# nikizadehgfdl/ocean_model_grid_generator

Measured on AMD Instinct MI355X. Metric: supergrid cells/sec (coords+metrics), 1/8° tripolar at 1/2/4/8 MI355X, higher is better.
Workload: dtype f64

## Files before the change

### include/ogg_hip.h

```cpp
#ifndef OGG_HIP_H
#define OGG_HIP_H

#ifdef __cplusplus
extern "C" {
#endif

#define OGG_OK 0
#define OGG_EORDER 1
#define OGG_ESHAPE 2
#define OGG_EHIP 3
#define OGG_ENOMEM 4
#define OGG_EARG 5

#define OGG_DP_ARC_LITERAL 0
#define OGG_DP_ARC_CHORD 1

#define OGG_SYM_DEFAULT 0
#define OGG_SYM_MIRROR 1
#define OGG_SYM_NONE 2

const char* ogg_last_error(void);
const char* ogg_version(void);
long ogg_abi_sizeof(int which);
int ogg_device_count(int* count);
int ogg_set_device(int device);
int ogg_device_name(char* buf, int buflen);


int ogg_y_mercator_rounded(long Ni, long n, const double* phi_rad, long long* ystar);
int ogg_y_mercator_rounded_dev(long Ni, long n, const double* phi_rad, long long* ystar, void* stream);

int ogg_y_mercator(long Ni, long n, const double* phi_rad, double* y);
int ogg_y_mercator_dev(long Ni, long n, const double* phi_rad, double* y, void* stream);

int ogg_phi_mercator(long Ni, long n, const double* y, double* phi_deg);
int ogg_phi_mercator_dev(long Ni, long n, const double* y, double* phi_deg, void* stream);
int ogg_mercator_axis_dev(long Ni, long long y0, long n, double* phi_deg, void* stream);

int ogg_linear_axis_dev(long n, double a0, double len, double denom, double* out, void* stream);

int ogg_affine_index(long n, const double* idx, double a0, double len, double denom, double* out);
int ogg_affine_index_dev(long n, const double* idx, double a0, double len, double denom, double* out, void* stream);

int ogg_tile_latlon(long nrows, long ni1, const double* lat1d, const double* lon1d, double* x, double* y);
int ogg_tile_latlon_dev(long nrows, long ni1, const double* lat1d, const double* lon1d, double* x, double* y,
                        void* stream);

int ogg_generate_latlon_grid(long lni, long lnj, double llon0, double llen_lon, double llat0, double llen_lat,
                             int skip_first_row, double* x, double* y);


int ogg_mdist(long n, const double* x1, const double* x2, double* out);
int ogg_mdist_dev(long n, const double* x1, const double* x2, double* out, void* stream);

int ogg_grid_metrics_midas_dev(long nrows_xy, long ni1, const double* x, const double* y, long n_pt_rows,
                               long n_cell_rows, double Re, int latlon_areafix, double* dx, double* dy,
                               double* area, double* angle, void* stream);
int ogg_grid_metrics_midas(long nj1, long ni1, const double* x, const double* y, double Re, int latlon_areafix,
                           double* dx, double* dy, double* area);
int ogg_angle_x(long nj1, long ni1, const double* x, const double* y, double* angle_dx);

typedef struct {
    int axis_kind;
    double a0, len, denom;
    long long y0;
    const double* lat1d;
    long k0;
    long n_pt_rows;
    long n_cell_rows;
    double *x, *y, *dx, *dy, *area, *angle;
} ogg_latlon_band;
int ogg_latlon_supergrid_multi_dev(int n_bands, const ogg_latlon_band* bands, long ni1, double lon0, double lenlon, double Re,
                                   int metrics, void* stream);
long ogg_latlon_rows_workspace_bytes(int n_bands, const ogg_latlon_band* bands, long ni1);
int ogg_latlon_supergrid_rows_ws_dev(int n_bands, const ogg_latlon_band* bands, long ni1, double lon0, double lenlon, double Re,
                                     int metrics, void* workspace, long workspace_bytes, void* stream);
int ogg_latlon_supergrid_dev(long n_pt_rows, long n_cell_rows, long ni1, const double* lat1d, const double* lon1d, double Re,
                             int metrics, double* x, double* y, double* dx, double* dy, double* area, double* angle,
                             void* stream);


int ogg_bipolar_projection(long n, const double* lamg, const double* phig, double lon_bp, double rp,
                           int metrics_only, double* lams, double* phis, double* h_i_inv, double* h_j_inv);
int ogg_bipolar_projection_dev(long n, const double* lamg, const double* phig, double lon_bp, double rp,
                               int metrics_only, double* lams, double* phis, double* h_i_inv, double* h_j_inv,
                               void* stream);

int ogg_bipolar_cap_mesh_dev(long Ni, long Nj, double lat0_bp, double lon_bp, long j0, long nrows, double* lams,
                             double* phis, double* h_i_inv, double* h_j_inv, void* stream);
int ogg_bipolar_cap_mesh_angle_dev(long Ni, long Nj, double lat0_bp, double lon_bp, long j0, long nrows, double* lams,
                                   double* phis, double* h_i_inv, double* h_j_inv, double* angle_dx, void* stream);
int ogg_bipolar_cap_mesh_angle_sym_dev(long Ni, long Nj, double lat0_bp, double lon_bp, long j0, long nrows, int symmetry, double* lams,
                                       double* phis, double* h_i_inv, double* h_j_inv, double* angle_dx, void* stream);
int ogg_bipolar_cap_mesh(long Ni, long Nj, double lat0_bp, double lon_bp, double* lams, double* phis,
                         double* h_i_inv, double* h_j_inv);
int ogg_bipolar_cap_mesh_sym(long Ni, long Nj, double lat0_bp, double lon_bp, int symmetry, double* lams, double* phis,
                             double* h_i_inv, double* h_j_inv);

int ogg_bipolar_cap_ij_array(long n_i, const double* i, long n_j, const double* j, long Ni, long Nj, double lat0_bp,
                             double lon_bp, double rp, double* h_i_inv, double* h_j_inv);
int ogg_bipolar_cap_ij_array_dev(long n_i, const double* i, long n_j, const double* j, long Ni, long Nj, double lat0_bp,
                                 double lon_bp, double rp, double* h_i_inv, double* h_j_inv, void* stream);

int ogg_bipolar_cap_metrics_quad_dev(int order, long nx, long ny, double lat0_bp, double lon_bp, double rp,
                                     double Re, long j0, long n_dx_rows, long n_cell_rows, double* dxq, double* dyq,
                                     double* daq, void* stream);
int ogg_bipolar_cap_metrics_quad(int order, long nx, long ny, double lat0_bp, double lon_bp, double rp, double Re,
                                 double* dxq, double* dyq, double* daq);
int ogg_bipolar_cap_metrics_quad_sym(int order, long nx, long ny, double lat0_bp, double lon_bp, double rp, double Re, int symmetry,
                                     double* dxq, double* dyq, double* daq);
long ogg_bipolar_quad_workspace_bytes(int order, long nx, long ny);
int ogg_bipolar_cap_metrics_quad_ws_dev(int order, long nx, long ny, double lat0_bp, double lon_bp, double rp, double Re,
                                        long j0, long n_dx_rows, long n_cell_rows, double* dxq, double* dyq, double* daq,
                                        void* workspace, long workspace_bytes, void* stream);
int ogg_bipolar_cap_metrics_quad_sym_ws_dev(int order, long nx, long ny, double lat0_bp, double lon_bp, double rp, double Re,
                                            long j0, long n_dx_rows, long n_cell_rows, int symmetry, double* dxq, double* dyq, double* daq,
                                            void* workspace, long workspace_bytes, void* stream);

typedef struct ogg_bipolar_band {
    long Ni, Nj;
    double lat0_bp, lon_bp;
    double rp, Re;
    int order;
    int symmetry;
    long j0;
    long n_pt_rows;
    long n_cell_rows;
    double *x, *y, *angle, *dx, *dy, *area;
    void* workspace;
// ... 474 lines not shown
```

### ocean_model_grid_generator_amd/_lib.py

```python
import ctypes
import os

import numpy as np

_HERE = os.path.dirname(os.path.abspath(__file__))
LIB_PATH = os.environ.get("OGG_LIB_PATH") or os.path.join(_HERE, "csrc", "libogg_hip.so")

OGG_OK, OGG_EORDER, OGG_ESHAPE, OGG_EHIP, OGG_ENOMEM, OGG_EARG = 0, 1, 2, 3, 4, 5
DP_ARC_LITERAL, DP_ARC_CHORD = 0, 1
SYM_DEFAULT, SYM_MIRROR, SYM_NONE = 0, 1, 2

MATH = {"div_pi180": 0, "rcp_c3": 1, "rsqrt_c3": 2, "atan_series14": 3, "atan_series17": 4, "atan_cap": 5, "atan2_angle": 6,
        "wave_prev": 7, "wave_next": 8, "wave_prev_tail": 9, "wave_next_tail": 10, "xcd_contiguous": 11, "lib_atan": 12, "atan_lib": 13, "wave_next_int": 14,
        "sin_tiny": 32, "asin_tiny": 33, "cos_cap": 34, "hom_arc": 35, "hom_tan": 36, "lib_sin": 37, "lib_asin": 38, "lib_cos": 39}

c_long, c_int, c_double, c_void_p, c_longlong = ctypes.c_long, ctypes.c_int, ctypes.c_double, ctypes.c_void_p, ctypes.c_longlong
_dp = ctypes.POINTER(ctypes.c_double)
_llp = ctypes.POINTER(ctypes.c_longlong)

class LatlonBand(ctypes.Structure):
    _fields_ = [("axis_kind", c_int), ("a0", c_double), ("len", c_double), ("denom", c_double), ("y0", c_longlong),
                ("lat1d", c_void_p), ("k0", c_long), ("n_pt_rows", c_long), ("n_cell_rows", c_long), ("x", c_void_p),
                ("y", c_void_p), ("dx", c_void_p), ("dy", c_void_p), ("area", c_void_p), ("angle", c_void_p)]

# ... 227 lines not shown
                                         c_void_p, c_void_p, c_void_p, c_void_p],
    "ogg_bipolar_cap_metrics_quad_ws_dev": [c_int, c_long, c_long, c_double, c_double, c_double, c_double, c_long, c_long, c_long,
                                            c_void_p, c_void_p, c_void_p, c_void_p, c_long, c_void_p],
    "ogg_bipolar_cap_metrics_quad_sym_ws_dev": [c_int, c_long, c_long, c_double, c_double, c_double, c_double, c_long, c_long, c_long, c_int,
                                                c_void_p, c_void_p, c_void_p, c_void_p, c_long, c_void_p],
    "ogg_bipolar_cap_metrics_quad": [c_int, c_long, c_long, c_double, c_double, c_double, c_double, c_void_p, c_void_p,
                                     c_void_p],
    "ogg_displaced_pole_mesh_dev": [c_long, c_void_p, c_long, c_void_p, c_long, c_long, c_double, c_double, c_double,
                                    c_double, c_void_p, c_void_p, c_void_p],
    "ogg_displaced_pole_mesh": [c_long, c_void_p, c_long, c_void_p, c_long, c_long, c_double, c_double, c_double, c_double,
                                c_void_p, c_void_p],
    "ogg_displaced_pole_grid_dev": [c_long, c_long, c_double, c_double, c_double, c_double, c_long, c_long, c_void_p,
                                    c_void_p, c_void_p],
    "ogg_displaced_pole_numerical_h_dev": [c_long, c_void_p, c_long, c_void_p, c_long, c_long, c_double, c_double, c_double,
                                           c_double, c_double, c_int, c_void_p, c_void_p, c_void_p],
    "ogg_displaced_pole_numerical_h": [c_long, c_void_p, c_long, c_void_p, c_long, c_long, c_double, c_double, c_double,
                                       c_double, c_double, c_int, c_void_p, c_void_p],
    "ogg_displaced_pole_metrics_quad_dev": [c_int, c_long, c_long, c_double, c_double, c_double, c_double, c_double, c_long,
                                            c_long, c_long, c_void_p, c_void_p, c_void_p, c_void_p],
    "ogg_displaced_pole_metrics_quad_ws_dev": [c_int, c_long, c_long, c_double, c_double, c_double, c_double, c_double, c_long,
                                               c_long, c_long, c_void_p, c_void_p, c_void_p, c_void_p, c_long, c_void_p],
    "ogg_displaced_pole_metrics_quad": [c_int, c_long, c_long, c_double, c_double, c_double, c_double, c_double, c_void_p,
                                        c_void_p, c_void_p],
    "ogg_displaced_pole_metrics_quad_form": [c_int, c_int, c_long, c_long, c_double, c_double, c_double, c_double, c_double, c_void_p,
                                             c_void_p, c_void_p],
    "ogg_displaced_pole_metrics_quad_form_ws_dev": [c_int, c_int, c_long, c_long, c_double, c_double, c_double, c_double, c_double,
                                                    c_long, c_long, c_long, c_void_p, c_void_p, c_void_p, c_void_p, c_long, c_void_p],
    "ogg_displaced_pole_metrics_quad_form_sym_ws_dev": [c_int, c_int, c_int, c_long, c_long, c_double, c_double, c_double, c_double, c_double,
                                                        c_long, c_long, c_long, c_void_p, c_void_p, c_void_p, c_void_p, c_long, c_void_p],
    "ogg_displaced_pole_grid_angle_ws_dev": [c_long, c_long, c_double, c_double, c_double, c_double, c_long, c_long, c_void_p,
                                             c_void_p, c_void_p, c_void_p, c_long, c_void_p],
    "ogg_workspace_error_flag_dev": [c_void_p, ctypes.POINTER(c_int), c_void_p],
    "ogg_y_mercator": [c_long, c_long, c_void_p, c_void_p],
    "ogg_y_mercator_dev": [c_long, c_long, c_void_p, c_void_p, c_void_p],
    "ogg_affine_index": [c_long, c_void_p, c_double, c_double, c_double, c_void_p],
    "ogg_affine_index_dev": [c_long, c_void_p, c_double, c_double, c_double, c_void_p, c_void_p],
    "ogg_mdist": [c_long, c_void_p, c_void_p, c_void_p],
    "ogg_mdist_dev": [c_long, c_void_p, c_void_p, c_void_p, c_void_p],
    "ogg_haversine": [c_long, c_void_p, c_void_p, c_void_p, c_void_p, c_void_p],
    "ogg_haversine_dev": [c_long, c_void_p, c_void_p, c_void_p, c_void_p, c_void_p, c_void_p],
    "ogg_bipolar_cap_ij_array": [c_long, c_void_p, c_long, c_void_p, c_long, c_long, c_double, c_double, c_double, c_void_p,
                                 c_void_p],
    "ogg_bipolar_cap_ij_array_dev": [c_long, c_void_p, c_long, c_void_p, c_long, c_long, c_double, c_double, c_double,
                                     c_void_p, c_void_p, c_void_p],
    "ogg_displaced_pole_projection": [c_long, c_long, c_void_p, c_void_p, c_double, c_double, c_double, c_double, c_void_p,
                                      c_void_p],
    "ogg_displaced_pole_projection_dev": [c_long, c_long, c_void_p, c_void_p, c_double, c_double, c_double, c_double,
                                          c_void_p, c_void_p, c_void_p],
    "ogg_monotonic_bounding": [c_long, c_long, c_void_p, c_double],
    "ogg_monotonic_bounding_dev": [c_long, c_long, c_void_p, c_double, c_void_p],
    "ogg_latlon_supergrid_multi_dev": [c_int, ctypes.POINTER(LatlonBand), c_long, c_double, c_double, c_double, c_int, c_void_p],
    "ogg_latlon_supergrid_rows_ws_dev": [c_int, ctypes.POINTER(LatlonBand), c_long, c_double, c_double, c_double, c_int, c_void_p, c_long,
                                         c_void_p],
    "ogg_tripolar_pass_dev": [c_int, ctypes.POINTER(LatlonBand), c_long, c_double, c_double, c_double, c_int,
                              ctypes.POINTER(BipolarBand), c_void_p],
    "ogg_tripolar_pass_events_dev": [c_int, ctypes.POINTER(LatlonBand), c_long, c_double, c_double, c_double, c_int,
                                     ctypes.POINTER(BipolarBand), ctypes.POINTER(c_void_p), ctypes.POINTER(c_double), c_void_p],
    "ogg_supergrid_pass_dev": [c_int, ctypes.POINTER(LatlonBand), c_long, c_double, c_double, c_double, c_int,
                               ctypes.POINTER(BipolarBand), ctypes.POINTER(DpoleBand), ctypes.POINTER(c_void_p), ctypes.POINTER(c_double),
                               c_void_p],
    "ogg_supergrid_pass_plan_dev": [c_int, ctypes.POINTER(LatlonBand), c_long, c_double, c_double, c_double, c_int,
                                    ctypes.POINTER(BipolarBand), ctypes.POINTER(DpoleBand), ctypes.POINTER(c_void_p)],
    "ogg_supergrid_pass_run_dev": [c_void_p, ctypes.POINTER(c_void_p), ctypes.POINTER(c_double), c_void_p],
    "ogg_supergrid_pass_plan_destroy": [c_void_p],
    "ogg_supergrid_pass_plan_flags_dev": [c_void_p, ctypes.POINTER(c_int), c_void_p],
    "ogg_latlon_supergrid_dev": [c_long, c_long, c_long, c_void_p, c_void_p, c_double, c_int, c_void_p, c_void_p, c_void_p,
                                 c_void_p, c_void_p, c_void_p, c_void_p],
    "ogg_fill_dev": [c_long, c_double, c_void_p, c_void_p],
    "ogg_bswap64_dev": [c_long, c_void_p, c_void_p, c_void_p],
    "ogg_libm_check_dev": [c_int, c_long, c_void_p, c_void_p, c_void_p, c_void_p],
    "ogg_math_eval_dev": [c_int, c_long, c_void_p, c_void_p, c_void_p, c_void_p],
    "ogg_metrics_sums_dev": [c_long, c_long, c_long, c_void_p, c_void_p, c_void_p, c_long, c_long, c_int, c_int, c_void_p, c_void_p],
    "ogg_grid_quality_band_dev": [ctypes.POINTER(QualityBand), c_void_p, c_long, c_void_p, c_void_p],
    "ogg_grid_quality": [ctypes.POINTER(QualityBand), ctypes.POINTER(QualityResult)],
    "ogg_topog_band_dev": [ctypes.POINTER(TopogBand), ctypes.POINTER(TopogSource), c_void_p, c_long, c_void_p, c_void_p],
    "ogg_topog_quantize_dev": [ctypes.POINTER(TopogSource), c_void_p, c_void_p, c_void_p],
    "ogg_topog": [ctypes.POINTER(TopogBand), ctypes.POINTER(TopogSource), c_void_p],
    "ogg_topog_plane_band_dev": [ctypes.POINTER(TopogBand), ctypes.POINTER(TopogSource), c_void_p, c_long, c_void_p, c_void_p],
    "ogg_topog_plane": [ctypes.POINTER(TopogBand), ctypes.POINTER(TopogSource), c_void_p],
    "ogg_xgrid_check_atm": [ctypes.POINTER(XgridAtm)],
    "ogg_xgrid_count_dev": [ctypes.POINTER(XgridBand), ctypes.POINTER(XgridAtm), c_void_p, c_long, c_void_p, c_void_p, c_void_p],
    "ogg_xgrid_write_dev": [ctypes.POINTER(XgridBand), ctypes.POINTER(XgridAtm), c_void_p, c_long, c_void_p, c_void_p, c_void_p,
                            c_void_p],
    "ogg_xgrid": [ctypes.POINTER(XgridBand), ctypes.POINTER(XgridAtm), c_long, c_void_p, c_void_p, c_void_p, c_void_p,
                  ctypes.POINTER(XgridCounts)],
    "ogg_mask_check": [ctypes.POINTER(MaskParams)],
    "ogg_mask_label_dev": [ctypes.POINTER(MaskParams), c_void_p, c_void_p, c_long, c_void_p, c_void_p, c_void_p, c_void_p],
    "ogg_mask_seed_dev": [ctypes.POINTER(MaskParams), c_void_p, c_void_p, c_long, c_int, c_void_p, c_void_p, c_void_p],
    "ogg_mask_apply_dev": [ctypes.POINTER(MaskParams), c_void_p, c_void_p, c_void_p, c_long, c_void_p, c_int, c_void_p, c_void_p,
                           c_void_p, c_void_p],
    "ogg_ocean_mask": [ctypes.POINTER(MaskParams), c_void_p, c_void_p, c_void_p, c_int, c_void_p, c_void_p, c_void_p, c_void_p,
                       c_void_p, c_void_p, c_long, ctypes.POINTER(MaskCounts)],
    "ogg_remap_check": [ctypes.POINTER(RemapParams)],
    "ogg_remap_segments_dev": [ctypes.POINTER(RemapParams), c_void_p, c_long, c_void_p, c_long, c_void_p],
    "ogg_remap_dev": [ctypes.POINTER(RemapParams), c_void_p, c_void_p, c_void_p, c_long, c_void_p, c_void_p, c_long, c_void_p, c_void_p,
                      c_void_p, c_void_p],
    "ogg_remap_fill_dev": [ctypes.POINTER(RemapParams), c_void_p, c_long, c_void_p, c_void_p, c_void_p, c_void_p],
    "ogg_remap": [ctypes.POINTER(RemapParams), c_void_p, c_void_p, c_void_p, c_void_p, c_long, c_void_p, c_int, c_void_p, c_void_p,
                  ctypes.POINTER(RemapCounts)],
    "ogg_runoff_check": [ctypes.POINTER(RunoffParams)],
    "ogg_runoff_targets_dev": [ctypes.POINTER(RunoffParams), c_void_p, c_void_p, c_long, c_void_p, c_void_p, c_long, c_void_p, c_void_p,
                               c_void_p, c_void_p],
    "ogg_runoff_sources_dev": [ctypes.POINTER(RunoffParams), c_void_p, c_void_p, c_void_p, c_void_p, c_long, c_void_p, c_void_p, c_void_p,
                               c_void_p, c_void_p],
    "ogg_runoff_search_dev": [ctypes.POINTER(RunoffParams), c_void_p, c_void_p, c_long, c_void_p, c_long, c_void_p, c_long, c_void_p,
                              c_void_p, c_void_p, c_void_p],
    "ogg_runoff_segments_dev": [ctypes.POINTER(RunoffParams), c_void_p, c_long, c_void_p, c_long, c_void_p],
    "ogg_runoff_accumulate_dev": [ctypes.POINTER(RunoffParams), c_void_p, c_void_p, c_long, c_void_p, c_long, c_void_p, c_long, c_void_p,
                                  c_void_p, c_void_p, c_void_p],
    "ogg_runoff": [ctypes.POINTER(RunoffParams), c_void_p, c_void_p, c_void_p, c_void_p, c_void_p, c_void_p, c_void_p, c_void_p, c_void_p,
                   c_void_p, c_void_p, c_void_p, ctypes.POINTER(RunoffCounts)],
    "ogg_coast_check": [ctypes.POINTER(CoastParams)],
    "ogg_coast_sets_dev": [ctypes.POINTER(CoastParams), c_void_p, c_void_p, c_long, c_void_p, c_void_p, c_long, c_void_p, c_void_p, c_void_p,
                           c_void_p, c_void_p, c_void_p, c_void_p, c_void_p],
    "ogg_coast_search_dev": [ctypes.POINTER(CoastParams), c_void_p, c_void_p, c_void_p, c_void_p, c_long, c_void_p, c_void_p, c_long,
                             c_void_p, c_long, c_void_p, c_void_p, c_void_p, c_void_p],
    "ogg_coast_distance": [ctypes.POINTER(CoastParams), c_void_p, c_void_p, c_void_p, c_void_p, c_void_p, c_void_p,
                           ctypes.POINTER(CoastCounts)],
    "ogg_basin_check": [ctypes.POINTER(BasinParams), c_void_p],
    "ogg_basin_plan": [ctypes.POINTER(BasinParams), c_void_p, c_void_p, ctypes.POINTER(c_int)],
    "ogg_basin_codes_dev": [ctypes.POINTER(BasinParams), c_void_p, c_void_p, c_void_p, c_void_p, c_long, c_void_p, c_void_p, c_long,
                            c_void_p, c_void_p, c_void_p, c_void_p, c_void_p],
    "ogg_basin_codes": [ctypes.POINTER(BasinParams), c_void_p, c_void_p, c_void_p, c_void_p, c_void_p, c_void_p, c_void_p,
                        ctypes.POINTER(BasinCounts)],
    "ogg_regrid_check": [ctypes.POINTER(RegridParams)],
    "ogg_regrid_transpose_dev": [ctypes.POINTER(RegridParams), c_void_p, c_void_p, c_void_p, c_long, c_void_p, c_long, c_void_p, c_void_p],
    "ogg_regrid_dev": [ctypes.POINTER(RegridParams), c_void_p, c_void_p, c_long, c_void_p, c_long, c_void_p, c_void_p, c_void_p, c_void_p,
                       c_void_p, c_void_p],
    "ogg_regrid": [ctypes.POINTER(RegridParams), c_void_p, c_void_p, c_void_p, c_void_p, c_long, c_void_p, c_void_p, c_void_p, c_void_p,
                   c_void_p, ctypes.POINTER(RegridCounts)],
    "ogg_bilinear_check": [ctypes.POINTER(BilinearParams), c_int],
    "ogg_bilinear_dev": [ctypes.POINTER(BilinearParams), c_void_p, c_void_p, c_long, c_void_p, c_void_p, c_void_p, c_void_p, c_void_p,
                         c_void_p, c_void_p, c_void_p, c_void_p, c_void_p, c_void_p, c_void_p],
    "ogg_bilinear_rotate_dev": [ctypes.POINTER(BilinearParams), c_void_p, c_long, c_void_p, c_void_p, c_void_p, c_void_p, c_void_p,
                                c_void_p, c_void_p, c_void_p, c_void_p, c_void_p, c_int, c_void_p],
    "ogg_bilinear": [ctypes.POINTER(BilinearParams), c_void_p, c_void_p, c_void_p, c_void_p, c_void_p, c_void_p, c_void_p, c_void_p, c_int,
                     c_int, c_void_p, c_void_p, c_void_p, c_void_p, c_void_p, c_void_p, c_void_p, c_void_p],
    "ogg_event_create": [ctypes.POINTER(c_void_p)],
    "ogg_event_destroy": [c_void_p],
    "ogg_event_record": [c_void_p, c_void_p],
    "ogg_event_elapsed_ms": [c_void_p, c_void_p, ctypes.POINTER(ctypes.c_float)],
    "ogg_stream_synchronize": [c_void_p],
}
STRING_GETTERS = ("ogg_last_error", "ogg_version")
LONG_GETTERS = {"ogg_abi_sizeof": [c_int],
                "ogg_bipolar_quad_workspace_bytes": [c_int, c_long, c_long],
                "ogg_displaced_pole_quad_workspace_bytes": [c_int, c_long, c_long],
                "ogg_displaced_pole_grid_workspace_bytes": [c_long, c_long],
                "ogg_dpole_band_workspace_bytes": [c_int, c_long, c_long],
                "ogg_latlon_rows_workspace_bytes": [c_int, ctypes.POINTER(LatlonBand), c_long],
                "ogg_supergrid_pass_plan_slots": [c_void_p],
                "ogg_supergrid_pass_plan_carried_runs": [c_void_p],
                "ogg_grid_quality_result_bytes": [],
                "ogg_grid_quality_workspace_bytes": [c_long, c_long],
                "ogg_topog_record_bytes": [],
                "ogg_topog_plane_record_bytes": [],
                "ogg_topog_band_out_rows": [ctypes.POINTER(TopogBand)],
                "ogg_topog_workspace_bytes": [],
                "ogg_xgrid_struct_bytes": [c_int],
                "ogg_xgrid_band_first_row": [ctypes.POINTER(XgridBand)],
                "ogg_xgrid_band_out_rows": [ctypes.POINTER(XgridBand)],
                "ogg_xgrid_band_next_rows": [ctypes.POINTER(XgridBand)],
                "ogg_xgrid_workspace_bytes": [ctypes.POINTER(XgridBand), ctypes.POINTER(XgridAtm)],
                "ogg_mask_struct_bytes": [c_int],
                "ogg_mask_workspace_bytes": [ctypes.POINTER(MaskParams)],
                "ogg_remap_struct_bytes": [c_int],
                "ogg_remap_workspace_bytes": [ctypes.POINTER(RemapParams)],
                "ogg_runoff_struct_bytes": [c_int],
                "ogg_runoff_workspace_bytes": [ctypes.POINTER(RunoffParams)],
                "ogg_coast_struct_bytes": [c_int],
                "ogg_coast_workspace_bytes": [ctypes.POINTER(CoastParams)],
                "ogg_basin_struct_bytes": [c_int],
                "ogg_basin_workspace_bytes": [ctypes.POINTER(BasinParams)],
                "ogg_regrid_struct_bytes": [c_int],
                "ogg_regrid_workspace_bytes": [ctypes.POINTER(RegridParams), c_long],
                "ogg_bilinear_struct_bytes": []}

_lib = None


class OggHipError(Exception):

    def __init__(self, code, text):
        Exception.__init__(self, text)
        self.code = code


def load():
    global _lib
    if _lib is not None:
        return _lib
    if not os.path.exists(LIB_PATH):
        raise ImportError("libogg_hip.so is not built (%s). Run `python -m ocean_model_grid_generator_amd.csrc.build` "
                          "(needs hipcc); this package has no CPU fallback." % LIB_PATH)
    if not os.environ.get("OGG_NO_TORCH"):
        try:
            import torch
        except ImportError:
            pass
    lib = ctypes.CDLL(LIB_PATH)
    for name, argtypes in SIGNATURES.items():
        if os.environ.get("OGG_LIB_PATH") and not hasattr(lib, name):
            continue
# ... 55 lines not shown
```

### ocean_model_grid_generator_amd/csrc/ogg_latlon_fused.hip

```cpp
#include "ogg_latlon_fused_dev.h"

namespace {

struct RowsParams {
    FusedParams f;
    const RowScalars* row_tab;
    long row0[LF_MAX_BANDS + 1];
    const double* col_tab;
    long unit0[LF_MAX_BANDS * 6 + 1];
};

__global__ __launch_bounds__(256) void latlon_tables_kernel(RowsParams p) {
    const long k = (long)blockIdx.x * blockDim.x + threadIdx.x;
    const FusedParams& f = p.f;
    const long n_rows = p.row0[f.n_bands];
    if (k < n_rows) {
        int bi = 0;
        while (bi + 1 < f.n_bands && k >= p.row0[bi + 1]) ++bi;
        const_cast<RowScalars*>(p.row_tab)[k] = latlon_row_scalars(f, f.band[bi], k - p.row0[bi]);
    } else if (k < n_rows + f.ni1) {
        const long i = k - n_rows;
        const ColScalars c = column_scalars(f, i);
        double* t = const_cast<double*>(p.col_tab);
        t[i] = c.lon_c, t[f.ni1 + i] = c.dlam, t[2 * f.ni1 + i] = c.hdlam, t[3 * f.ni1 + i] = c.xdiff;
// ... 56 lines not shown
    if (n_bands < 0 || n_bands > LF_MAX_BANDS || (n_bands && !bands) || ni1 < 2) return 0;
    long rows = 0;
    for (int k = 0; k < n_bands; ++k) rows += (bands[k].n_pt_rows > 0 ? bands[k].n_pt_rows : 0) + 1;
    return rows * (long)sizeof(RowScalars) + 4 * ni1 * (long)sizeof(double);
}

extern "C" int ogg_latlon_supergrid_rows_ws_dev(int n_bands, const ogg_latlon_band* bands, long ni1, double lon0, double lenlon, double Re,
                                                int metrics, void* workspace, long workspace_bytes, void* stream) {
    RowsParams r{};
    long points = 0;
    if (int e = plan_latlon(n_bands, bands, ni1, lon0, lenlon, Re, metrics, r.f, points)) return e;
    if (r.f.n_bands == 0) return OGG_OK;
    OGG_REQUIRE(workspace && workspace_bytes >= ogg_latlon_rows_workspace_bytes(n_bands, bands, ni1), OGG_EARG,
                "ogg_latlon_supergrid_rows: workspace too small (ogg_latlon_rows_workspace_bytes)");
    r.row0[0] = 0, r.unit0[0] = 0;
    for (int k = 0; k < r.f.n_bands; ++k) {
        const ogg_latlon_band& b = r.f.band[k];
        r.row0[k + 1] = r.row0[k] + b.n_pt_rows + 1;
        const long ncell = metrics ? b.n_cell_rows : 0;
        const long rows_of[6] = {b.n_pt_rows, b.n_pt_rows, b.n_pt_rows, metrics ? b.n_pt_rows : 0, ncell, ncell};
        for (int fld = 0; fld < 6; ++fld) r.unit0[k * 6 + fld + 1] = r.unit0[k * 6 + fld] + rows_of[fld];
    }
    r.row_tab = static_cast<const RowScalars*>(workspace);
    r.col_tab = reinterpret_cast<const double*>(r.row_tab + r.row0[r.f.n_bands]);
    hipStream_t st = ogg::as_stream(stream);
    const long n_tab = r.row0[r.f.n_bands] + ni1;
    latlon_tables_kernel<<<(unsigned)((n_tab + 255) / 256), 256, 0, st>>>(r);
    OGG_LAUNCH_CHECK();
    long max_wg = 1 << 20;
    if (const char* e = getenv("OGG_ROWS_MAX_WG")) max_wg = atol(e) > 0 ? atol(e) : max_wg;
    const long n_units = r.unit0[r.f.n_bands * 6];
    latlon_rows_kernel<<<(unsigned)(n_units < max_wg ? n_units : max_wg), 256, 0, st>>>(r);
    OGG_LAUNCH_CHECK();
    return OGG_OK;
}

extern "C" int ogg_latlon_supergrid_multi_dev(int n_bands, const ogg_latlon_band* bands, long ni1, double lon0, double lenlon,
                                              double Re, int metrics, void* stream) {
    FusedParams p;
    long points = 0;
    if (int e = plan_latlon(n_bands, bands, ni1, lon0, lenlon, Re, metrics, p, points)) return e;
    if (p.n_bands == 0) return OGG_OK;
    const long gx = latlon_gx(ni1);
    long max_wg = 240;
    if (const char* e = getenv("OGG_FUSED_MAX_WG")) max_wg = atol(e);
    long gy = p.strip0[p.n_bands];
    if (gx * gy > max_wg) gy = (max_wg + gx - 1) / gx;
    dim3 grid((unsigned)gx, (unsigned)(gy < 1 ? 1 : gy));
    latlon_fused_kernel<<<grid, LF_TX, 0, ogg::as_stream(stream)>>>(p);
    OGG_LAUNCH_CHECK();
    return OGG_OK;
}

extern "C" int ogg_latlon_supergrid_dev(long n_pt_rows, long n_cell_rows, long ni1, const double* lat1d, const double* lon1d,
                                        double Re, int metrics, double* x, double* y, double* dx, double* dy, double* area,
                                        double* angle, void* stream) {
    OGG_REQUIRE(lat1d && lon1d, OGG_EARG, "ogg_latlon_supergrid: null axis");
    double ends[2];
    OGG_HIP_CHECK(hipMemcpyAsync(&ends[0], lon1d, sizeof(double), hipMemcpyDeviceToHost, ogg::as_stream(stream)));
    OGG_HIP_CHECK(hipMemcpyAsync(&ends[1], lon1d + (ni1 - 1), sizeof(double), hipMemcpyDeviceToHost, ogg::as_stream(stream)));
    OGG_HIP_CHECK(hipStreamSynchronize(ogg::as_stream(stream)));
    ogg_latlon_band b{};
    b.axis_kind = 2, b.lat1d = lat1d, b.k0 = 0, b.n_pt_rows = n_pt_rows, b.n_cell_rows = n_cell_rows;
    b.x = x, b.y = y, b.dx = dx, b.dy = dy, b.area = area, b.angle = angle;
    return ogg_latlon_supergrid_multi_dev(1, &b, ni1, ends[0], ends[1] - ends[0], Re, metrics, stream);
}
```

### ocean_model_grid_generator_amd/csrc/ogg_latlon_fused_dev.h

```cpp
#pragma once
#include <cmath>
#include <cstdlib>

#include "../../include/ogg_hip.h"
#include "ogg_common.h"
#include "ogg_math.h"

namespace {
using namespace ogg;

constexpr int LF_TX = 256;
constexpr int LF_ROWS = 32;
constexpr int LF_MAX_BANDS = 4;

struct RowScalars {
    double lat, sl, cl, dy;
};

struct FusedParams {
    int n_bands;
    ogg_latlon_band band[LF_MAX_BANDS];
    long strip0[LF_MAX_BANDS + 1];
    long ni1;
    double lon0, lenlon, Ni;
// ... 80 lines not shown
            if (first) q[0] = a;
            if (second) q[1] = b;
        }
    }
}

OGG_DEV double latlon_angle(double pa) {
    const double r = (__double2hiint(pa) < 0) ? kPi / kPi180 : 0.0 / kPi180;
    return (pa != pa) ? pa : r;
}

template <bool FULL, bool NT>
OGG_DEV void latlon_rows(const FusedParams& p, const ogg_latlon_band& b, const RowScalars* s_row, long js, int nrows, long n_cell_rows,
                         long i0, const ColScalars& c0, const ColScalars& c1) {
    const long ni1 = p.ni1, ni = ni1 - 1;
    const bool pt1 = i0 + 1 < ni1, ce0 = i0 < ni;
    double* __restrict__ px = b.x + (js * ni1 + i0);
    double* __restrict__ py = b.y + (js * ni1 + i0);
    double* __restrict__ pa = b.angle + (js * ni1 + i0);
    double* __restrict__ pdx = b.dx + (js * ni + i0);
    double* __restrict__ pdy = b.dy + (js * ni1 + i0);
    double* __restrict__ par = b.area + (js * ni + i0);
    for (int r = 0; r < nrows; ++r) {
        const long j = js + r;
        const RowScalars rs = s_row[r];
        store2<FULL, NT>(px, c0.lon_c, c1.lon_c, true, pt1);
        store2<FULL, NT>(py, rs.lat, rs.lat, true, pt1);
        store2<FULL, NT>(pa, latlon_angle(c0.xdiff * rs.cl), latlon_angle(c1.xdiff * rs.cl), true, pt1);
        if (p.metrics) {
            store2<FULL, NT>(pdx, p.Re * fabs(c0.dlam * rs.cl), p.Re * fabs(c1.dlam * rs.cl), ce0, false);
            if (j < n_cell_rows) {
                store2<FULL, NT>(pdy, rs.dy, rs.dy, true, pt1);
                const double ds = s_row[r + 1].sl - rs.sl;
                store2<FULL, NT>(par, p.Re2 * (c0.hdlam * ds), p.Re2 * (c1.hdlam * ds), ce0, false);
            }
        }
        px += ni1, py += ni1, pa += ni1, pdy += ni1;
        pdx += ni, par += ni;
    }
}

OGG_DEV unsigned ticket_ask(unsigned* counter) {
    unsigned ret;
    const unsigned one = 1u;
    asm volatile("global_atomic_add %0, %1, %2, off sc0" : "=v"(ret) : "v"(counter), "v"(one) : "memory");
    return ret;
}
template <int LATER>
OGG_DEV unsigned ticket_answer(unsigned pending) {
    unsigned out;
    asm volatile("s_waitcnt vmcnt(%2)\n\tv_mov_b32 %0, %1" : "=v"(out) : "v"(pending), "n"(LATER) : "memory");
    return out;
}

constexpr int LF_COLS = 2 * LF_TX;
inline long latlon_gx(long ni1) { return (ni1 + LF_COLS - 1) / LF_COLS; }

template <bool NT, bool TAB = false>
OGG_DEV void latlon_fused_body(const FusedParams& p, RowScalars* s_row, long b, long gx, long gy, long strip_lo, long strip_hi,
                               unsigned* claims = nullptr, bool helper = false, int* s_claim = nullptr, bool pool = false) {
    const long v = xcd_contiguous(b, gx * gy);
    const long bx = v % gx, by = v / gx;
    const int tid = threadIdx.x;
    const long i0 = (bx * LF_TX + tid) * 2;
    const long ni1 = p.ni1, ni = ni1 - 1;
    const ColScalars c0 = column_scalars(p, i0), c1 = column_scalars(p, i0 + 1);
    const bool full = i0 + 1 < ni;
    const long per = (strip_hi - strip_lo + gy - 1) / gy;
    const long s_first = strip_lo + by * per, s_last = (s_first + per < strip_hi) ? s_first + per : strip_hi;
    unsigned* cnt = claims ? (pool ? claims + bx : claims + 2 * (by * gx + bx)) : nullptr;
    const unsigned n_pool = (unsigned)(strip_hi - strip_lo);
    if (pool) {
        if (tid == 0) {
            const unsigned t = atomicAdd(cnt, 1u);
            *s_claim = t < n_pool ? (int)t : -1;
        }
        __syncthreads();
    }
    long walked = 0;
    for (long strip = s_first;; ++strip) {
        unsigned asked;
        if (pool) {
            const int pick = *s_claim;
            if (pick < 0) break;
            strip = strip_lo + pick;
            if (tid == 0) asked = ticket_ask(cnt);
        } else if (cnt) {
            if (tid == 0) {
                const unsigned n = (unsigned)(s_last > s_first ? s_last - s_first : 0);
                int pick = -1;
                if (atomicAdd(cnt, 1u) < n) pick = helper ? (int)(n - 1u - atomicAdd(cnt + 1, 1u)) : (int)walked;
                *s_claim = pick;
            }
            __syncthreads();
            const int pick = *s_claim;
            if (pick < 0) break;
            strip = s_first + pick;
            ++walked;
        } else if (strip >= s_last) {
            break;
        }
        int bi = 0;
        while (bi + 1 < p.n_bands && strip >= p.strip0[bi + 1]) ++bi;
        const ogg_latlon_band& b = p.band[bi];
        const long n_cell_rows = p.metrics ? b.n_cell_rows : 0;
        const long js = (strip - p.strip0[bi]) * p.rows_per_block;
        const long je = (js + p.rows_per_block < b.n_pt_rows) ? js + p.rows_per_block : b.n_pt_rows;
        const int nrows = (int)(je - js);
        if (TAB) {
            if (tid <= nrows) s_row[tid] = p.row_tab[p.row0[bi] + js + tid];
        } else {
            if (tid <= nrows) {
                const long j = js + tid;
                const bool have = (tid < nrows) || (j - 1 < n_cell_rows);
                RowScalars r = {0.0, 0.0, 0.0, 0.0};
                if (have) {
                    r.lat = axis_lat(b, b.k0 + j, p.Ni);
                    const double lv = (0.5 * (r.lat + r.lat)) * kPi180;
                    sincos(lv, &r.sl, &r.cl);
                }
                s_row[tid] = r;
            }
            __syncthreads();
            if (p.metrics && tid < nrows) {
                const long j = js + tid;
                if (j < n_cell_rows) {
                    const double dyj = (s_row[tid + 1].lat - s_row[tid].lat) * kPi180;
                    s_row[tid].dy = p.Re * sqrt(dyj * dyj + 0.0);
                }
            }
        }
        __syncthreads();
        if (full)
            latlon_rows<true, NT>(p, b, s_row, js, nrows, n_cell_rows, i0, c0, c1);
        else if (i0 < ni1)
            latlon_rows<false, NT>(p, b, s_row, js, nrows, n_cell_rows, i0, c0, c1);
        if (pool && tid == 0) {
            const unsigned t = nrows >= 6 ? ticket_answer<16>(asked) : nrows == 5 ? ticket_answer<12>(asked) : nrows == 4 ? ticket_answer<8>(asked)
                               : nrows == 3 ? ticket_answer<6>(asked) : ticket_answer<0>(asked);
            *s_claim = t < n_pool ? (int)t : -1;
        }
        __syncthreads();
    }
}

__global__ __launch_bounds__(LF_TX) void latlon_fused_kernel(FusedParams p) {
    __shared__ RowScalars s_row[LF_ROWS + 1];
    latlon_fused_body<false>(p, s_row, (long)blockIdx.y * gridDim.x + blockIdx.x, gridDim.x, gridDim.y, 0, p.strip0[p.n_bands]);
}

inline void set_rows_per_strip(FusedParams& p, long rpb) {
    rpb = rpb < 1 ? 1 : (rpb > LF_ROWS ? LF_ROWS : rpb);
    p.rows_per_block = (int)rpb;
    p.strip0[0] = 0;
    for (int k = 0; k < p.n_bands; ++k) p.strip0[k + 1] = p.strip0[k] + (p.band[k].n_pt_rows + rpb - 1) / rpb;
}

inline int plan_latlon(int n_bands, const ogg_latlon_band* bands, long ni1, double lon0, double lenlon, double Re, int metrics,
                       FusedParams& p, long& points) {
    OGG_REQUIRE(n_bands >= 0 && n_bands <= LF_MAX_BANDS && (n_bands == 0 || bands) && ni1 >= 2, OGG_EARG,
                "ogg_latlon_supergrid_multi: bad argument (at most %d bands)", LF_MAX_BANDS);
    p = FusedParams{};
    long total_rows = 0;
    points = 0;
    for (int k = 0; k < n_bands; ++k) {
        const ogg_latlon_band& b = bands[k];
        OGG_REQUIRE(b.n_pt_rows >= 0 && b.n_cell_rows >= 0 && b.n_cell_rows <= b.n_pt_rows, OGG_ESHAPE,
                    "ogg_latlon_supergrid_multi: band %d rows pt=%ld cell=%ld", k, b.n_pt_rows, b.n_cell_rows);
        if (b.n_pt_rows == 0) continue;
        OGG_REQUIRE(b.x && b.y && b.angle && (b.axis_kind != 2 || b.lat1d), OGG_EARG, "ogg_latlon_supergrid_multi: null pointer in band %d", k);
        OGG_REQUIRE(!metrics || (b.dx && (b.n_cell_rows == 0 || (b.dy && b.area))), OGG_EARG,
                    "ogg_latlon_supergrid_multi: null metrics output in band %d", k);
        p.band[p.n_bands++] = b;
        total_rows += b.n_pt_rows;
        points += b.n_pt_rows * ni1;
    }
    if (p.n_bands == 0) return OGG_OK;
    const long gx = latlon_gx(ni1);
    long rpb = (total_rows * gx + 2047) / 2048;
    rpb = rpb < 8 ? 8 : (rpb > LF_ROWS ? LF_ROWS : rpb);
    if (const char* e = getenv("OGG_LL_ROWS_PER_STRIP")) rpb = atol(e) < 1 ? 1 : (atol(e) > LF_ROWS ? LF_ROWS : atol(e));
    p.row0[0] = 0;
    for (int k = 0; k < p.n_bands; ++k) p.row0[k + 1] = p.row0[k] + p.band[k].n_pt_rows + 1;
    p.ni1 = ni1, p.lon0 = lon0, p.lenlon = lenlon, p.Ni = (double)(ni1 - 1);
    p.Re = Re, p.Re2 = pow(Re, 2.0), p.metrics = metrics;
    set_rows_per_strip(p, rpb);
    return OGG_OK;
}

}
```

### ocean_model_grid_generator_amd/supergrid.py

```python
import ctypes
import math
import os

import numpy as np

from . import _lib as L
from . import ocean_grid_generator as ogg

FIELDS = ("x", "y", "dx", "dy", "area", "angle_dx")


def band(n_rows, rank, world):
    return (n_rows * rank) // world, (n_rows * (rank + 1)) // world


def band_weighted(cost, rank, world, top_capacity=1.0, capacities=None):
    c = np.concatenate(([0.0], np.cumsum(np.asarray(cost, dtype=np.float64))))
    total = c[-1]
    caps = [1.0] * (world - 1) + [float(top_capacity)] if capacities is None else [float(v) for v in capacities]
    if len(caps) != world or min(caps) <= 0.0:
        raise ValueError("band_weighted: %d capacities for %d ranks (all must be positive)" % (len(caps), world))
    before = np.concatenate(([0.0], np.cumsum(caps)))

    def edge(r):
# ... 312 lines not shown
                raise Exception("--south_cutoff_ang reads the southern cap's latitudes (OGG:1278): there is no southern cap")
            if sc_y0 is None:
                if first.kind != "latlon":
                    raise ValueError("south_cut: the cap's latitudes are needed for --south_cutoff_ang")
                sc_y0 = first.lat0 + (np.arange(first.row0, first.row0 + first.nj1) * first.lenlat) / float(first.lnj)
            jcut = 1 + int(np.nonzero(np.asarray(sc_y0) < self.south_cutoff_ang)[0][-1])
        else:
            return 0, 0, False
        if has_sc and jcut < n_sc:
            if (n_sc - jcut) % 2 == 0 and self.ensure_nj_even:
                jcut += 1
            return jcut, 0, False
        so = next((s for s in self.subs if s.name == "SO"), None)
        if so is None:
            return 0, 0, False
        if not has_sc:
            raise Exception("--south_cutoff_row without a southern cap: the reference reads lamSC here (OGG:1299)")
        jcut_so = jcut - n_sc
        if (so.nj1 - 1 - jcut_so - 1) % 2 == 0 and self.ensure_nj_even:
            jcut_so += 1
        return n_sc, jcut_so, True

    def rows_cut(self, sc_y0=None):
        c_sc, c_so, gone = self.south_cut(sc_y0)
        if not gone:
            return c_sc
        so = next(s for s in self.subs if s.name == "SO")
        return self.subs[0].nj1 - 1 + min(c_so, so.nj1 - 1)

    @property
    def nyp(self):
        return sum(s.nj1 - 1 for s in self.subs) + 1 - self.rows_cut()

    @property
    def cells(self):
        return (self.nyp - 1) * self.Ni


class Supergrid(object):

    def __init__(self, plan, rank=0, world=1, device="cuda:0", halo="rccl", peers=None, latlon="fused"):
        import torch

        self.torch = torch
        self.plan, self.rank, self.world, self.halo, self.latlon = plan, rank, world, halo, latlon
        self.device = torch.device(device)
        self.peers = peers
        self.overlap = True
        self.launch = "pass" if latlon == "fused" else "kernels"
        self.pass_events = None
        self._event_pool = []
        self._pass_args = None
        self._rows_ws = None
        self._side = None
        self.buf = {}
        self.timings = {}
        ni1 = plan.Ni + 1
        import contextlib
        with (torch.cuda.device(self.device) if self.device.type == "cuda" else contextlib.nullcontext()):
            self.lon1d = torch.empty(ni1, dtype=torch.float64, device=self.device)
            def field_shapes():
                for s in plan.subs:
                    lo, hi = self.rows_of(s, rank, world)
                    n = hi - lo
                    n_cell = max(min(hi, s.nj1 - 1) - lo, 0)
                    halo = 1 if (latlon == "stencil" and s.kind in ("mercator", "latlon") and n_cell > 0 and hi < s.nj1) else 0
                    for r, c in ((n + halo, ni1), (n + halo, ni1), (n, ni1 - 1), (n_cell, ni1), (n_cell, ni1 - 1), (n, ni1)):
                        yield max(r, 0) * c * 8

            slab, slab_off, slab_align = None, 0, 0
            if self.device.type == "cuda":
                forced = os.environ.get("OGG_FIELD_SLAB")
                sizes = list(field_shapes())
                if forced is not None:
                    slab_align = int(forced)
                if slab_align > 0:
                    total = sum((b + slab_align - 1) // slab_align * slab_align for b in sizes) + slab_align
                    try:
                        free_bytes = torch.cuda.mem_get_info(self.device)[0]
                    except Exception:
                        free_bytes = 0
                    if total > free_bytes * 9 // 10:
                        slab_align = 0
                    else:
                        slab = torch.empty(total, dtype=torch.uint8, device=self.device)
                        slab_off = (-slab.data_ptr()) % slab_align
                        self._slab = slab
            self.field_slab = {"spacing_bytes": slab_align, "bytes": int(slab.numel()) if slab is not None else 0}

            def field_buffer(r, c):
                nonlocal slab_off
                if slab is None:
                    return torch.empty((max(r, 0), c), dtype=torch.float64, device=self.device)
                nbytes = max(r, 0) * c * 8
                t = slab[slab_off:slab_off + nbytes].view(torch.float64).view(max(r, 0), c)
                slab_off += (nbytes + slab_align - 1) // slab_align * slab_align
                return t

            for s in plan.subs:
                lo, hi = self.rows_of(s, rank, world)
                n = hi - lo
                n_cell = min(hi, s.nj1 - 1) - lo
                needs_halo = latlon == "stencil" and s.kind in ("mercator", "latlon") and n_cell > 0 and hi < s.nj1
                b = {"lo": lo, "hi": hi, "n": n, "n_cell": max(n_cell, 0), "needs_halo": needs_halo}
                rows_xy = n + (1 if needs_halo else 0)
                for f, (r, c) in (("x", (rows_xy, ni1)), ("y", (rows_xy, ni1)), ("dx", (n, ni1 - 1)), ("dy", (b["n_cell"], ni1)),
# ... 140 lines not shown
        self.replan()

    def __del__(self):
        try:
            self.replan()
        except Exception:
            pass

    @staticmethod
    def _new_events():
        evs = (ctypes.c_void_p * 5)()
        for k in range(5):
            e = ctypes.c_void_p()
            L.call("ogg_event_create", ctypes.byref(e))
            evs[k] = e
        return evs

    def reserve_pass_events(self, n):
        self._event_pool = [self._new_events() for _ in range(n)]

    def pass_launch_times_ms(self):
        L.call("ogg_stream_synchronize", self._stream())
        tot = [0.0, 0.0, 0.0, 0.0]
        n = len(self.pass_events)
        for evs in self.pass_events:
            for k in range(4):
                ms = ctypes.c_float()
                L.call("ogg_event_elapsed_ms", evs[k], evs[k + 1], ctypes.byref(ms))
                tot[k] += ms.value
            for k in range(5):
                L.call("ogg_event_destroy", evs[k])
        self.pass_events = []
        by = list(self.pass_bytes) if n else [0.0, 0.0, 0.0, 0.0]
        out = {name: {"ms": tot[k] / max(n, 1), "alg_bytes": by[k]} for k, name in enumerate(("pass_a", "pass_b", "pass_tail", "pass_dpquad"))}
        out["sampled_passes"] = n
        return out

    def phase_a(self, only=None, kinds=None):
        p, st = self.plan, self._stream()
        ni1 = p.Ni + 1
        if only is None and self.latlon != "fused":
            L.call("ogg_linear_axis_dev", ni1, p.lon0, p.lenlon, float(p.Ni), self.lon1d.data_ptr(), st)
        if self.latlon == "fused":
            bands = self._latlon_bands(only, kinds)
            if bands:
                import os
                arr = (L.LatlonBand * len(bands))(*bands)
                if os.environ.get("OGG_LATLON_ROWS", "0") != "0":
                    need = int(L.load().ogg_latlon_rows_workspace_bytes(len(bands), arr, ni1))
                    if self._rows_ws is None or self._rows_ws.numel() < need:
                        self._rows_ws = self.torch.empty(need, dtype=self.torch.uint8, device=self.device)
                    ws = self._rows_ws
                    self._timed("latlon_fused", lambda: L.call("ogg_latlon_supergrid_rows_ws_dev", len(bands), arr, ni1, p.lon0, p.lenlon,
                                                               p.Re, 0 if p.skip_metrics else 1, ws.data_ptr(), ws.numel(), st))
                else:
                    self._timed("latlon_fused", lambda: L.call("ogg_latlon_supergrid_multi_dev", len(bands), arr, ni1, p.lon0, p.lenlon,
                                                               p.Re, 0 if p.skip_metrics else 1, st))
        for s in p.subs:
            b = self.buf[s.name]
            if b["n"] == 0 or not self._selected(s, only, kinds):
                continue
            if s.kind in ("mercator", "latlon"):
                if self.latlon == "fused":
                    continue
                if s.kind == "mercator":
                    if getattr(s, "explicit_axis", None) is None:
                        L.call("ogg_mercator_axis_dev", p.Ni, s.y0, s.n_axis, b["axis"].data_ptr(), st)
                else:
                    L.call("ogg_linear_axis_dev", s.lnj + 1, s.lat0, s.lenlat, float(s.lnj), b["axis"].data_ptr(), st)
                rows = b["n"] + (1 if (b["needs_halo"] and self.halo == "recompute") else 0)
                self._timed("tile_latlon", lambda: L.call("ogg_tile_latlon_dev", rows, ni1, self._p(b["axis"], s.row0 + b["lo"]),
                                                          self.lon1d.data_ptr(), b["x"].data_ptr(), b["y"].data_ptr(), st))
            elif s.kind == "bipolar":
                if hasattr(L.load(), "ogg_bipolar_cap_mesh_angle_sym_dev"):
                    self._timed("bipolar_mesh", lambda: L.call("ogg_bipolar_cap_mesh_angle_sym_dev", p.Ni, s.Nj, s.lat0_bp, s.lon_bp, b["lo"], b["n"],
                                                               p.cap_symmetry, b["x"].data_ptr(), b["y"].data_ptr(), None, None,
                                                               b["angle_dx"].data_ptr(), st))
                else:
                    self._timed("bipolar_mesh", lambda: L.call("ogg_bipolar_cap_mesh_angle_dev", p.Ni, s.Nj, s.lat0_bp, s.lon_bp, b["lo"], b["n"],
                                                               b["x"].data_ptr(), b["y"].data_ptr(), None, None, b["angle_dx"].data_ptr(), st))
            elif s.kind == "dpole":
                self._timed("dpole_mesh", lambda: L.call("ogg_displaced_pole_grid_angle_ws_dev", p.Ni, s.Nj, p.lon0, s.lat0, s.lon_dp, s.r_dp,
                                                         s.row0 + b["lo"], b["n"], b["x"].data_ptr(), b["y"].data_ptr(),
                                                         b["angle_dx"].data_ptr(), b["ws"].data_ptr(), b["ws_mesh_bytes"], st))

    def exchange_halo(self):
        if self.world == 1 or self.halo == "recompute" or self.latlon == "fused":
            return
        torch = self.torch
        if self.halo == "local":
            for s in self.plan.subs:
                b = self.buf[s.name]
                if b["needs_halo"]:
                    up = self.peers[self.rank + 1].buf[s.name]
                    b["x"][b["n"]].copy_(up["x"][0])
                    b["y"][b["n"]].copy_(up["y"][0])
            return
        import torch.distributed as dist

        ops = []
        for s in self.plan.subs:
            if s.kind not in ("mercator", "latlon"):
                continue
            b = self.buf[s.name]
            if b["needs_halo"]:
                ops.append(dist.P2POp(dist.irecv, b["x"][b["n"]], self.rank + 1))
# ... 742 lines not shown
```

Before: 125.8 billion.

## Add workspace-backed strip-claiming latlon kernel with precomputed row table

Adds a new latlon fused path that first fills a per-row scalar table and zeroes claim counters in a separate kernel. A second kernel then uses a fixed-size grid of workgroups (108 by default) that claim row strips dynamically from that table. The Python side selects this path by default when the library provides it, and it caches the workspace across calls. The aim is to avoid recomputing row scalars per block and to balance work across a persistent grid, at the cost of an extra launch and atomic claim traffic.

```diff
diff --git a/include/ogg_hip.h b/include/ogg_hip.h
--- a/include/ogg_hip.h
+++ b/include/ogg_hip.h
@@ -75,6 +75,9 @@
 long ogg_latlon_rows_workspace_bytes(int n_bands, const ogg_latlon_band* bands, long ni1);
 int ogg_latlon_supergrid_rows_ws_dev(int n_bands, const ogg_latlon_band* bands, long ni1, double lon0, double lenlon, double Re,
                                      int metrics, void* workspace, long workspace_bytes, void* stream);
+long ogg_latlon_strips_workspace_bytes(int n_bands, const ogg_latlon_band* bands, long ni1);
+int ogg_latlon_supergrid_multi_ws_dev(int n_bands, const ogg_latlon_band* bands, long ni1, double lon0, double lenlon, double Re,
+                                      int metrics, void* workspace, long workspace_bytes, void* stream);
 int ogg_latlon_supergrid_dev(long n_pt_rows, long n_cell_rows, long ni1, const double* lat1d, const double* lon1d, double Re,
                              int metrics, double* x, double* y, double* dx, double* dy, double* area, double* angle,
                              void* stream);
diff --git a/ocean_model_grid_generator_amd/_lib.py b/ocean_model_grid_generator_amd/_lib.py
--- a/ocean_model_grid_generator_amd/_lib.py
+++ b/ocean_model_grid_generator_amd/_lib.py
@@ -303,6 +303,8 @@
     "ogg_latlon_supergrid_multi_dev": [c_int, ctypes.POINTER(LatlonBand), c_long, c_double, c_double, c_double, c_int, c_void_p],
     "ogg_latlon_supergrid_rows_ws_dev": [c_int, ctypes.POINTER(LatlonBand), c_long, c_double, c_double, c_double, c_int, c_void_p, c_long,
                                          c_void_p],
+    "ogg_latlon_supergrid_multi_ws_dev": [c_int, ctypes.POINTER(LatlonBand), c_long, c_double, c_double, c_double, c_int, c_void_p, c_long,
+                                          c_void_p],
     "ogg_tripolar_pass_dev": [c_int, ctypes.POINTER(LatlonBand), c_long, c_double, c_double, c_double, c_int,
                               ctypes.POINTER(BipolarBand), c_void_p],
     "ogg_tripolar_pass_events_dev": [c_int, ctypes.POINTER(LatlonBand), c_long, c_double, c_double, c_double, c_int,
@@ -400,6 +402,7 @@
                 "ogg_displaced_pole_grid_workspace_bytes": [c_long, c_long],
                 "ogg_dpole_band_workspace_bytes": [c_int, c_long, c_long],
                 "ogg_latlon_rows_workspace_bytes": [c_int, ctypes.POINTER(LatlonBand), c_long],
+                "ogg_latlon_strips_workspace_bytes": [c_int, ctypes.POINTER(LatlonBand), c_long],
                 "ogg_supergrid_pass_plan_slots": [c_void_p],
                 "ogg_supergrid_pass_plan_carried_runs": [c_void_p],
                 "ogg_grid_quality_result_bytes": [],
diff --git a/ocean_model_grid_generator_amd/csrc/ogg_latlon_fused.hip b/ocean_model_grid_generator_amd/csrc/ogg_latlon_fused.hip
--- a/ocean_model_grid_generator_amd/csrc/ogg_latlon_fused.hip
+++ b/ocean_model_grid_generator_amd/csrc/ogg_latlon_fused.hip
@@ -132,6 +132,62 @@
     return OGG_OK;
 }
 
+namespace {
+
+__global__ __launch_bounds__(LF_TX) void latlon_strips_table_kernel(FusedParams p, unsigned* claims, long gx) {
+    latlon_row_table_body(p, blockIdx.x, gridDim.x);
+    for (long k = (long)blockIdx.x * LF_TX + threadIdx.x; k < gx; k += (long)gridDim.x * LF_TX) claims[k] = 0u;
+}
+
+template <bool NT>
+__global__ __launch_bounds__(LF_TX) void latlon_strips_kernel(FusedParams p, unsigned* claims, long gx, long gy) {
+    __shared__ RowScalars s_row[LF_ROWS + 1];
+    __shared__ int s_claim;
+    latlon_fused_body<NT, true>(p, s_row, blockIdx.x, gx, gy, 0, p.strip0[p.n_bands], claims, false, &s_claim, true);
+}
+
+long strips_table_bytes(long rows) { return ogg::round256(rows * (long)sizeof(RowScalars)); }
+long strips_claim_bytes(long ni1) { return ogg::round256(latlon_gx(ni1) * (long)sizeof(unsigned)); }
+
+}
+
+extern "C" long ogg_latlon_strips_workspace_bytes(int n_bands, const ogg_latlon_band* bands, long ni1) {
+    if (n_bands < 0 || n_bands > LF_MAX_BANDS || (n_bands && !bands) || ni1 < 2) return 0;
+    long rows = 0;
+    for (int k = 0; k < n_bands; ++k)
+        if (bands[k].n_pt_rows > 0) rows += bands[k].n_pt_rows + 1;
+    return strips_table_bytes(rows) + strips_claim_bytes(ni1);
+}
+
+extern "C" int ogg_latlon_supergrid_multi_ws_dev(int n_bands, const ogg_latlon_band* bands, long ni1, double lon0, double lenlon,
+                                                 double Re, int metrics, void* workspace, long workspace_bytes, void* stream) {
+    FusedParams p;
+    long points = 0;
+    if (int e = plan_latlon(n_bands, bands, ni1, lon0, lenlon, Re, metrics, p, points)) return e;
+    if (p.n_bands == 0) return OGG_OK;
+    const long tab_bytes = strips_table_bytes(p.row0[p.n_bands]);
+    OGG_REQUIRE(workspace && workspace_bytes >= tab_bytes + strips_claim_bytes(ni1) && reinterpret_cast<unsigned long long>(workspace) % 16 == 0,
+                OGG_EARG, "ogg_latlon_supergrid_multi_ws: workspace too small or not 16-byte aligned (ogg_latlon_strips_workspace_bytes)");
+    int wg, rows, nt, max_wg;
+    if (int e = ogg::knob("OGG_FUSED_WS_WG", 108, 1, 1 << 20, &wg)) return e;
+    if (int e = ogg::knob("OGG_FUSED_WS_ROWS", 8, 1, LF_ROWS, &rows)) return e;
+    if (int e = ogg::knob("OGG_FUSED_WS_NT", 0, 0, 1, &nt)) return e;
+    if (int e = ogg::knob("OGG_FUSED_MAX_WG", 1 << 20, 1, 1 << 20, &max_wg)) return e;
+    set_rows_per_strip(p, rows);
+    p.row_tab = static_cast<const RowScalars*>(workspace);
+    unsigned* claims = ogg::at<unsigned>(workspace, tab_bytes);
+    const long gx = latlon_gx(ni1), gy = ((wg < max_wg ? wg : max_wg) + gx - 1) / gx;
+    hipStream_t st = ogg::as_stream(stream);
+    latlon_strips_table_kernel<<<(unsigned)latlon_row_table_blocks(p), LF_TX, 0, st>>>(p, claims, gx);
+    OGG_LAUNCH_CHECK();
+    if (nt)
+        latlon_strips_kernel<true><<<(unsigned)(gx * gy), LF_TX, 0, st>>>(p, claims, gx, gy);
+    else
+        latlon_strips_kernel<false><<<(unsigned)(gx * gy), LF_TX, 0, st>>>(p, claims, gx, gy);
+    OGG_LAUNCH_CHECK();
+    return OGG_OK;
+}
+
 extern "C" int ogg_latlon_supergrid_dev(long n_pt_rows, long n_cell_rows, long ni1, const double* lat1d, const double* lon1d,
                                         double Re, int metrics, double* x, double* y, double* dx, double* dy, double* area,
                                         double* angle, void* stream) {
diff --git a/ocean_model_grid_generator_amd/csrc/ogg_latlon_fused_dev.h b/ocean_model_grid_generator_amd/csrc/ogg_latlon_fused_dev.h
--- a/ocean_model_grid_generator_amd/csrc/ogg_latlon_fused_dev.h
+++ b/ocean_model_grid_generator_amd/csrc/ogg_latlon_fused_dev.h
@@ -156,6 +156,12 @@
     asm volatile("s_waitcnt vmcnt(%2)\n\tv_mov_b32 %0, %1" : "=v"(out) : "v"(pending), "n"(LATER) : "memory");
     return out;
 }
+
+constexpr int LF_ROW_STORES = 3;
+constexpr int LF_WAIT_6 = 16, LF_WAIT_5 = 12, LF_WAIT_4 = 8, LF_WAIT_3 = 6;
+static_assert(LF_WAIT_6 <= 6 * LF_ROW_STORES && LF_WAIT_5 <= 5 * LF_ROW_STORES && LF_WAIT_4 <= 4 * LF_ROW_STORES &&
+                  LF_WAIT_3 <= 3 * LF_ROW_STORES,
+              "a counted ticket wait must not exceed the stores its strip is sure to issue");
 
 constexpr int LF_COLS = 2 * LF_TX;
 inline long latlon_gx(long ni1) { return (ni1 + LF_COLS - 1) / LF_COLS; }
@@ -240,8 +246,8 @@
         else if (i0 < ni1)
             latlon_rows<false, NT>(p, b, s_row, js, nrows, n_cell_rows, i0, c0, c1);
         if (pool && tid == 0) {
-            const unsigned t = nrows >= 6 ? ticket_answer<16>(asked) : nrows == 5 ? ticket_answer<12>(asked) : nrows == 4 ? ticket_answer<8>(asked)
-                               : nrows == 3 ? ticket_answer<6>(asked) : ticket_answer<0>(asked);
+            const unsigned t = nrows >= 6 ? ticket_answer<LF_WAIT_6>(asked) : nrows == 5 ? ticket_answer<LF_WAIT_5>(asked)
+                               : nrows == 4 ? ticket_answer<LF_WAIT_4>(asked) : nrows == 3 ? ticket_answer<LF_WAIT_3>(asked) : ticket_answer<0>(asked);
             *s_claim = t < n_pool ? (int)t : -1;
         }
         __syncthreads();
diff --git a/ocean_model_grid_generator_amd/supergrid.py b/ocean_model_grid_generator_amd/supergrid.py
--- a/ocean_model_grid_generator_amd/supergrid.py
+++ b/ocean_model_grid_generator_amd/supergrid.py
@@ -388,6 +388,7 @@
         self._event_pool = []
         self._pass_args = None
         self._rows_ws = None
+        self._strips_ws = None
         self._side = None
         self.buf = {}
         self.timings = {}
@@ -634,6 +635,13 @@
                         self._rows_ws = self.torch.empty(need, dtype=self.torch.uint8, device=self.device)
                     ws = self._rows_ws
                     self._timed("latlon_fused", lambda: L.call("ogg_latlon_supergrid_rows_ws_dev", len(bands), arr, ni1, p.lon0, p.lenlon,
+                                                               p.Re, 0 if p.skip_metrics else 1, ws.data_ptr(), ws.numel(), st))
+                elif os.environ.get("OGG_LATLON_WS", "1") != "0" and hasattr(L.load(), "ogg_latlon_supergrid_multi_ws_dev"):
+                    need = int(L.load().ogg_latlon_strips_workspace_bytes(len(bands), arr, ni1))
+                    if self._strips_ws is None or self._strips_ws.numel() < need:
+                        self._strips_ws = self.torch.empty(need, dtype=self.torch.uint8, device=self.device)
+                    ws = self._strips_ws
+                    self._timed("latlon_fused", lambda: L.call("ogg_latlon_supergrid_multi_ws_dev", len(bands), arr, ni1, p.lon0, p.lenlon,
                                                                p.Re, 0 if p.skip_metrics else 1, ws.data_ptr(), ws.numel(), st))
                 else:
                     self._timed("latlon_fused", lambda: L.call("ogg_latlon_supergrid_multi_dev", len(bands), arr, ni1, p.lon0, p.lenlon,
```

Result: no change. 127.8 billion (median of 5 runs) (+1.6%).
